# zlib-ng/minizip-ng

Measured on NVIDIA H100. Metric: deflate_l1_crc32_input_throughput, higher is better.
Workload: dtype u8

## Files before the change

minizip-ng_b200/csrc/deflate_kernel.cuh:

```cuda
#ifndef MZ_DEFLATE_KERNEL_CUH
#define MZ_DEFLATE_KERNEL_CUH

#include "mzcuda_common.cuh"

namespace mzc {

constexpr int DF_THREADS = 512;
constexpr int DF_WARPS = DF_THREADS / 32;
constexpr int DF_CHUNK_MAX = 65536;
constexpr int DF_UNIT = 32768;
constexpr int DF_SB = DF_UNIT;
constexpr int DF_SPAN = 8;
constexpr int DF_BATCH = DF_THREADS * DF_SPAN;
constexpr int DF_NBATCH = DF_UNIT / DF_BATCH;
constexpr int DF_MINMATCH = 4;
constexpr int DF_LOCKLEN = 8;
constexpr int DF_HASH_BITS = 13;
constexpr int DF_HASH_ENTRIES = 1 << DF_HASH_BITS;
constexpr int DF_STAGE_WORDS = DF_UNIT / 4 + 64;
constexpr int DF_HDR_WORDS = 96;

constexpr uint32_t DF_FLAG_FINAL = 1u;
constexpr uint32_t DF_FLAG_DICT = 2u;

constexpr int DF_OFF_IN = 0;
constexpr int DF_OFF_HASH = DF_OFF_IN + DF_UNIT + 64;
constexpr int DF_OFF_STAGE = DF_OFF_HASH;
constexpr int DF_OFF_REC = DF_OFF_HASH + DF_STAGE_WORDS * 4;
constexpr int DF_OFF_SPN = DF_OFF_REC + DF_NBATCH * DF_THREADS * 8;
constexpr int DF_SPAN_BYTES = DF_NBATCH * DF_THREADS * 10;
constexpr int DF_OFF_HIST = DF_OFF_REC + DF_SPAN_BYTES;
constexpr int DF_OFF_HIST2 = DF_OFF_HIST + (288 + 32) * 4;
constexpr int DF_OFF_CODE = DF_OFF_HIST2 + 256 * 4;
constexpr int DF_OFF_LENS = DF_OFF_CODE + (288 + 32) * 4;
constexpr int DF_OFF_BITS = DF_OFF_LENS + (288 + 32);
constexpr int DF_OFF_SCAN = DF_OFF_BITS + (288 + 32);
constexpr int DF_OFF_BB = DF_OFF_SCAN + 256 * 4;
constexpr int DF_OFF_MISC = DF_OFF_BB + 512 * 4;
constexpr int DF_OFF_SINK = DF_OFF_MISC + 32 * 4 + 16;
constexpr int DF_OFF_LSYM = DF_OFF_SINK + 32 * 4;
constexpr int DF_SMEM_BYTES = DF_OFF_LSYM + 256 * 2;
constexpr uint32_t DF_ZERO_SYM = 286;
static_assert(DF_HASH_ENTRIES * 4 <= DF_STAGE_WORDS * 4, "hash fits the staging region");
constexpr int DFH_PREV = 32768;
constexpr int DFH_HASH_BITS = 14;
constexpr int DFH_OFF_HASH = (DF_SMEM_BYTES + 15) & ~15;
constexpr int DFH_SMEM_BYTES = DFH_PREV + DFH_OFF_HASH + (4 << DFH_HASH_BITS);
static_assert(DFH_SMEM_BYTES <= 227 * 1024, "shared memory budget of the history variant");
static_assert(DF_SMEM_BYTES <= 113 * 1024, "shared memory budget for two CTAs per SM");

enum { MISC_CHUNK = 3, MISC_CARRY = 8  };

struct DeflateParams {
    const uint8_t *in;
    const uint64_t *in_off;
    const uint32_t *in_len;
    const uint8_t *flags;
    uint64_t total_len;
    uint32_t chunk_size;
    uint32_t nchunks;
    uint32_t last_flags;
    int32_t level;
    uint8_t *out;
    uint64_t slot_stride;
    uint32_t *out_len;
    uint32_t *work_counter;
};

__host__ __device__ inline uint64_t deflate_slot_bound(uint32_t chunk_size) {
    return (((uint64_t)chunk_size + 12ull * ((chunk_size + DF_SB - 1) / DF_SB + 1) + 64 + 15) & ~15ull);
}

__device__ __forceinline__ void length_symbol(uint32_t len, uint32_t &sym, uint32_t &ebits, uint32_t &eval) {
    const uint32_t l = len - 3;
    const uint32_t msb = 31u - (uint32_t)__clz((int)(l | 4u));
    uint32_t e = msb - 2;
    uint32_t sy = 4 * (e + 1) + ((l >> e) & 3u);
    uint32_t ev = l & ((1u << e) - 1u);
    sy = l < 8 ? l : sy;
    const bool top = len == 258;
    sym = top ? 28u : sy;
    ebits = top ? 0u : e;
    eval = top ? 0u : ev;
}
__device__ __forceinline__ void dist_symbol0(uint32_t d, uint32_t &sym, uint32_t &ebits) {
    uint32_t m = 31u - (uint32_t)__clz((int)(d | 1u));
    ebits = m > 0 ? m - 1 : 0u;
    sym = 2 * m + ((d >> ebits) & 1u);
}
__device__ __forceinline__ uint32_t len_extra_bits(uint32_t lsym) { return (lsym < 8 || lsym >= 28) ? 0u : (lsym >> 2) - 1; }
__device__ __forceinline__ uint32_t dist_extra_bits(uint32_t dsym) { return dsym < 4 ? 0u : (dsym >> 1) - 1; }

__device__ __forceinline__ uint32_t stage_word(uint32_t base, uint32_t pos, uint32_t k4) { return base + __umulhi(pos, 1u << 27) * k4; }

__device__ __forceinline__ void stage_put(uint32_t *stage, uint32_t pos, uint32_t v, uint32_t n) {
    if (n == 0) return;
    if (n < 32) v &= (1u << n) - 1;
    uint32_t w = pos >> 5, s = pos & 31;
    atomicOr(&stage[w], v << s);
    if (s + n > 32) atomicOr(&stage[w + 1], v >> (32 - s));
}

__device__ __forceinline__ void stage_or(const Smem &sm, uint32_t pos, uint32_t v, uint32_t n) {
    const uint32_t sh = pos & 31u, wa = DF_OFF_STAGE + ((pos >> 5) << 2);
    sm.red_or32(wa, v << sh);
    if (sh + n > 32) sm.red_or32(wa + 4, v >> (32 - sh));
}

struct BitWriter {
    Smem sm;
    uint64_t acc;
    uint32_t nb, wa;
    __device__ __forceinline__ void init(const Smem &s, uint32_t bitoff) {
        sm = s; wa = DF_OFF_STAGE + (bitoff >> 5) * 4; nb = bitoff & 31; acc = 0;
    }
    __device__ __forceinline__ void put(uint32_t v, uint32_t n) {
        acc |= (uint64_t)v << nb;
        nb += n;
        if (nb >= 32) {
            sm.red_or32(wa, (uint32_t)acc);
            acc >>= 32; nb -= 32; wa += 4;
        }
    }
    __device__ __forceinline__ uint32_t bitpos() const { return ((wa - (uint32_t)DF_OFF_STAGE) << 3) + nb; }
    __device__ __forceinline__ void finish() {
        if (nb > 0) sm.red_or32(wa, (uint32_t)acc);
        if (nb > 32) sm.red_or32(wa + 4, (uint32_t)(acc >> 32));
    }
};

__device__ inline uint32_t block_excl_sum(uint32_t v, uint32_t *scan, uint32_t &total) {
    uint32_t incl = warp_incl_sum(v);
    if (lane_id() == 31) scan[warp_id()] = incl;
    __syncthreads();
    if (warp_id() == 0) {
        uint32_t w = lane_id() < (unsigned)DF_WARPS ? scan[lane_id()] : 0u;
        uint32_t wi = warp_incl_sum(w);
        scan[32 + lane_id()] = wi - w;
        if (lane_id() == 31) scan[31] = wi;
    }
    __syncthreads();
    uint32_t res = scan[32 + warp_id()] + incl - v;
    total = scan[31];
    __syncthreads();
    return res;
}

enum { DF_PH_LOAD, DF_PH_PARSE, DF_PH_M0, DF_PH_COVER, DF_PH_T_M1, DF_PH_D, DF_PH_E_SCAN, DF_PH_F_M3, DF_PH_FLUSH, DF_PH_UNITS,
       DF_PH_D_STATS, DF_PH_D_SWEEP1, DF_PH_D_SWEEP2, DF_PH_D_KRAFT, DF_PH_D_CANON, DF_PH_D_PASSES, DF_PH_COLS = DF_PH_D_PASSES + 8 };
constexpr int DF_PH_ROWS = 1024;
#if defined(MZ_DF_PHASES) && !defined(MZ_EMU)
__device__ unsigned long long g_df_phases[DF_PH_ROWS][DF_PH_COLS];
#define DF_PHASE_BEGIN(t) unsigned long long t = clock64()
#define DF_PHASE(t, ph)                                                                        \
    do {                                                                                       \
        if (threadIdx.x == 0 && blockIdx.x < (unsigned)DF_PH_ROWS) {                           \
            const unsigned long long now_ = clock64();                                         \
            atomicAdd(&g_df_phases[blockIdx.x][ph], now_ - (t));                               \
            if ((ph) == DF_PH_LOAD) atomicAdd(&g_df_phases[blockIdx.x][DF_PH_UNITS], 1ull);   \
            (t) = now_;                                                                        \
        }                                                                                      \
    } while (0)
#define DF_PHASE_COUNT(col)                                                                                          \
    do {                                                                                                             \
        if (threadIdx.x == 0 && blockIdx.x < (unsigned)DF_PH_ROWS) atomicAdd(&g_df_phases[blockIdx.x][col], 1ull); \
    } while (0)
#else
#define DF_PHASE_BEGIN(t)
#define DF_PHASE(t, ph)
#define DF_PHASE_COUNT(col)
#endif

constexpr int DF_BB_THREADS = 320;
enum { BB_STAT = 0 , BB_KRAFT = 8 , BB_SLACK = 136 ,
       BB_CNTW = 144 ,
       BB_NZ = 464 , BB_ST = 474 ,
       BB_HSUM = 484 , BB_HDRBITS = 494  };

constexpr uint64_t CL_LENS = 0x12ddad91b725bb4ull;
constexpr uint64_t CL_CODE_LO = 0x840013930ef3c6ull, CL_CODE_HI = 0xd5c7fdf6cb149ull;
constexpr uint64_t CL_ORDER57 = 0x1b6d6db248db92dull;
__device__ __forceinline__ uint32_t cl_len(uint32_t s) { return (uint32_t)(CL_LENS >> (3 * s)) & 7u; }
__device__ __forceinline__ uint32_t cl_code(uint32_t s) {
    return s < 10 ? (uint32_t)(CL_CODE_LO >> (6 * s)) & 63u : (uint32_t)(CL_CODE_HI >> (6 * (s - 10))) & 63u;
}

__device__ __forceinline__ void bb_count_lengths(uint32_t *cntw_row, uint32_t L, unsigned lane, unsigned &m) {
    if (lane < 16) cntw_row[lane] = 0;
    __syncwarp();
    m = __match_any_sync(MZ_FULL_MASK, L);
    if (L > 0 && lane == (unsigned)(__ffs((int)m) - 1)) cntw_row[L] = (uint32_t)__popc(m);
    __syncwarp();
}

__device__ inline void block_build_codes(const uint32_t *hist_ll, const uint32_t *hist_lit2, const uint32_t *hist_d, uint8_t *lens_ll, uint8_t *lens_d,
                                         uint32_t *code_ll, uint32_t *code_d, uint8_t *bits_ll, uint8_t *bits_d, uint32_t *bb,
                                         uint32_t *stage, uint32_t hdrpos, uint32_t bfinal) {
    const uint32_t tid = threadIdx.x;
    const unsigned lane = lane_id(), w = warp_id();
    const int a = tid < 288 ? 0 : (tid < 320 ? 1 : 2);
    const uint32_t sym = a == 0 ? tid : tid - 288;
    const uint32_t nsym = a == 0 ? 286u : 30u;
    const int M = 15;
    const uint32_t one = 1u << M;
    const uint32_t w0 = a == 0 ? 0u : 9u;
    uint32_t c = (a < 2 && sym < nsym) ? (a == 0 ? hist_ll[sym] + (sym < 256 ? hist_lit2[sym] : 0u) : hist_d[sym]) : 0u;
    DF_PHASE_BEGIN(d_t);

    if (tid < 144) bb[tid] = (tid == BB_STAT + 2 || tid == BB_STAT + 6) ? 0xffffffffu : 0u;
    bar_sync(1, DF_BB_THREADS);
    if (a < 2) {
        uint32_t used_w = __reduce_add_sync(MZ_FULL_MASK, c ? 1u : 0u);
        uint32_t tot_w = __reduce_add_sync(MZ_FULL_MASK, c);
        uint32_t first_w = __reduce_min_sync(MZ_FULL_MASK, c ? sym : 0xffffffffu);
        if (lane == 0) {
            atomicAdd(&bb[BB_STAT + a * 4 + 0], used_w);
            atomicAdd(&bb[BB_STAT + a * 4 + 1], tot_w);
            atomicMin(&bb[BB_STAT + a * 4 + 2], first_w);
        }
    }
    bar_sync(1, DF_BB_THREADS);
    DF_PHASE(d_t, DF_PH_D_STATS);
    float ideal = 0.f;
    if (a < 2) {
        uint32_t used = bb[BB_STAT + a * 4 + 0], total = bb[BB_STAT + a * 4 + 1], fu = bb[BB_STAT + a * 4 + 2];
        if (used < 2) {
            uint32_t d0 = used == 0 ? 0u : (fu == 0 ? 1u : 0u);
            uint32_t d1 = used == 0 ? 1u : d0;
            if ((sym == d0 || sym == d1) && c == 0) c = 1;
            total += 2 - used;
        }
        if (c) ideal = __log2f((float)total) - __log2f((float)c);
// ... 130 lines not shown
        if (a == 0) {
            const uint32_t eb = sym >= 257 ? len_extra_bits(sym - 257) : 0u;
            lens_ll[sym] = (uint8_t)L;
            code_ll[sym] = cw | (eb << 20);
            bits_ll[sym] = (uint8_t)(L + eb);
        } else {
            lens_d[sym] = (uint8_t)L;
            code_d[sym] = cw;
            bits_d[sym] = (uint8_t)(L + dist_extra_bits(sym));
        }
    }
    const unsigned nz = __ballot_sync(MZ_FULL_MASK, L != 0);
    if (lane == 0) bb[BB_NZ + w] = nz;
    bar_sync(1, DF_BB_THREADS);
    DF_PHASE(d_t, DF_PH_D_CANON);
    const uint32_t hlit = 256u + 32u - (uint32_t)__clz((int)bb[BB_NZ + 8]);
    const uint32_t hdw = bb[BB_NZ + 9];
    const uint32_t hdist = hdw ? 32u - (uint32_t)__clz((int)hdw) : 1u;
    const uint32_t nlen = a == 0 ? hlit : hdist;
    const bool valid = sym < nlen;
    const uint32_t prevL = sym == 0 ? 0xffu : (a == 0 ? lens_ll[sym - 1] : lens_d[sym - 1]);
    const unsigned st = __ballot_sync(MZ_FULL_MASK, (valid && prevL != L) || sym == nlen);
    if (lane == 0) bb[BB_ST + w] = st;
    bar_sync(1, DF_BB_THREADS);
    uint32_t nb = 0, val = 0;
    if (valid) {
        uint32_t m = st & (0xffffffffu >> (31u - lane)), ww = w;
        while (m == 0) m = bb[BB_ST + --ww];
        const uint32_t s0 = (ww - w0) * 32u + 31u - (uint32_t)__clz((int)m);
        m = lane == 31 ? 0u : st & (0xfffffffeu << lane);
        ww = w;
        while (m == 0) m = bb[BB_ST + ++ww];
        const uint32_t e0 = (ww - w0) * 32u + (uint32_t)__ffs((int)m) - 1u;
        const uint32_t k = sym - s0, R = e0 - s0;
        uint32_t cs = L, ev = 0, eb = 0;
        bool tok = true;
        if (L == 0) {
            const uint32_t full = (R / 138u) * 138u, rem = R - full;
            if (k < full) { tok = k % 138u == 0; cs = 18; ev = 127; eb = 7; }
            else if (rem >= 11) { tok = k == full; cs = 18; ev = rem - 11; eb = 7; }
            else if (rem >= 3) { tok = k == full; cs = 17; ev = rem - 3; eb = 3; }
        } else if (k > 0) {
            const uint32_t k1 = k - 1, rest = R - 1, full = (rest / 6u) * 6u, rem = rest - full;
            if (k1 < full) { tok = k1 % 6u == 0; cs = 16; ev = 3; eb = 2; }
            else if (rem >= 3) { tok = k1 == full; cs = 16; ev = rem - 3; eb = 2; }
        }
        if (tok) {
            const uint32_t cl = cl_len(cs);
            nb = cl + eb;
            val = cl_code(cs) | (ev << cl);
        }
    }
    const uint32_t incl = warp_incl_sum(nb);
    if (lane == 31) bb[BB_HSUM + w] = incl;
    bar_sync(1, DF_BB_THREADS);
    uint32_t off = incl - nb, total = 0;
    for (uint32_t ww = 0; ww < 10; ww++) {
        const uint32_t t = bb[BB_HSUM + ww];
        off += ww < w ? t : 0u;
        total += t;
    }
    if (nb) stage_put(stage, hdrpos + 17 + 57 + off, val, nb);
    if (tid == 0) {
        stage_put(stage, hdrpos, bfinal | (2u << 1) | ((hlit - 257u) << 3) | ((hdist - 1u) << 8) | (15u << 13), 17);
        bb[BB_HDRBITS] = 17 + 57 + total;
    }
    if (tid == 32) stage_put(stage, hdrpos + 17, (uint32_t)CL_ORDER57, 32);
    if (tid == 64) stage_put(stage, hdrpos + 17 + 32, (uint32_t)(CL_ORDER57 >> 32), 25);
}

__device__ __forceinline__ uint32_t extend_match8(const Smem &sm, uint32_t c, uint32_t q, uint32_t maxlen) {
    uint32_t len = 8;
    while (len < maxlen) {
        uint32_t x = sm.ld32u(DF_OFF_IN, q + len) ^ sm.ld32u(DF_OFF_IN, c + len);
        if (x) {
            len += (uint32_t)(__ffs((int)x) - 1) >> 3;
            break;
        }
        len += 4;
    }
    return len < maxlen ? len : maxlen;
}

__device__ __forceinline__ uint32_t opaque4() { return blockDim.x / (uint32_t)(DF_THREADS / 4); }

template <bool HIST>
__device__ __forceinline__ uint32_t hash_addr(uint32_t v, uint32_t k4) {
    return (HIST ? DFH_OFF_HASH : DF_OFF_HASH) + __umulhi(v * 2654435761u, 1u << (HIST ? DFH_HASH_BITS : DF_HASH_BITS)) * k4;
}

__device__ __forceinline__ uint32_t rec_len(uint32_t r) { uint32_t l = (r >> 3) & 255u; return l ? l + 3 : 0u; }

__device__ __forceinline__ uint32_t fin_len(uint32_t m) { return ((m >> 4) & 255u) + 3u; }
__device__ __forceinline__ uint32_t fin_dist(uint32_t m) { return ((m >> 12) & 0x7fffu) + 1u; }
template <bool ONEM>
__device__ __forceinline__ void span_classify(const Smem &sm, uint32_t A, uint32_t B, uint32_t q0, uint32_t cover, uint32_t &F, uint32_t &MA,
                                              uint32_t &MB) {
    const uint32_t lit = (A >> 26) | ((B >> 26) << 6);
    const uint32_t crel = cover > q0 ? cover - q0 : 0u;
    const uint32_t cr8 = crel < 8 ? crel : 8u;
    uint32_t ex = 0;
    MA = MB = 0;
#pragma unroll
    for (int r = 0; r < (ONEM ? 1 : 2); r++) {
        const uint32_t R = r == 0 ? A : B;
        const uint32_t j = R & 7u, end = j + rec_len(R);
        const uint32_t s = j > crel ? j : crel;
        const uint32_t Lf = (end > s ? end : s) - s;
        const uint32_t P = (s < 8u ? s : 8u) & 7u;
        const uint32_t M = Lf >= 3 ? (((Lf << 4) + (0x80000000u - (3u << 4))) | P | ((R << 1) & (0x7fffu << 12))) : 0u;
        if (r == 0) MA = M;
        else MB = M;
        ex = Lf - 1u < 2u ? Lf : ex;
    }
    F = ((lit >> cr8) << cr8) | (ex << 8);
    if (ex) {
        const uint32_t p = DF_OFF_IN + q0 + crel;
        F |= sm.ld8(p) << 16;
        if (ex == 2) F |= sm.ld8(p + 1) << 24;
    }
}

__device__ __forceinline__ uint32_t match_symbols(const Smem &sm, uint32_t M) {
    uint32_t ds, db;
    const uint32_t lsv = sm.ld16(DF_OFF_LSYM + ((M >> 3) & 0x1feu));
    const uint32_t d = fin_dist(M) - 1;
    dist_symbol0(d, ds, db);
    sm.red_add32(DF_OFF_HIST + (257u + (lsv & 31u)) * 4, 1u);
    sm.red_add32(DF_OFF_HIST + (288u + ds) * 4, 1u);
    return 0x80000000u | ((M & 7u) << 28) | ((d & ((1u << db) - 1u)) << 15) | (ds << 10) | lsv;
}
__device__ __forceinline__ uint32_t match_bits(const Smem &sm, uint32_t M) {
    const uint32_t n = sm.ld8(DF_OFF_BITS + 257u + (M & 31u)) + sm.ld8(DF_OFF_BITS + 288u + ((M >> 10) & 31u));
    return M ? n : 0u;
}
__device__ __forceinline__ void put_match_bits(const Smem &sm, uint32_t pos, uint32_t M) {
    const uint32_t cwl = sm.ld32(DF_OFF_CODE + (257u + (M & 31u)) * 4);
    const uint32_t cwd = sm.ld32(DF_OFF_CODE + (288u + ((M >> 10) & 31u)) * 4);
    const uint32_t cl = (cwl >> 16) & 15u, cd = (cwd >> 16) & 15u;
    const uint32_t v1 = (cwl & 0x7fffu) | (((M >> 5) & 31u) << cl);
    const uint32_t n1 = cl + ((cwl >> 20) & 15u);
    const uint32_t v2 = (cwd & 0x7fffu) | (((M >> 15) & 0x1fffu) << cd);
    const uint64_t V = (uint64_t)v1 | ((uint64_t)v2 << n1);
    const uint32_t lo = (uint32_t)V, hi = (uint32_t)(V >> 32);
    const uint32_t wa = stage_word(DF_OFF_STAGE, pos, opaque4());
    const uint32_t w0 = __funnelshift_l(0u, lo, pos), w1 = __funnelshift_l(lo, hi, pos), w2 = __funnelshift_l(hi, 0u, pos);
    sm.red_or32(wa, w0);
    sm.red_or32(wa + 4, w1);
    if (w2) sm.red_or32(wa + 8, w2);
}

__device__ __forceinline__ uint32_t nth_parked(const uint32_t (&bm)[DF_NBATCH], uint32_t k, uint32_t warp) {
    uint32_t r = k, word = 0, bsel = 0;
    bool found = false;
#pragma unroll
    for (int b = 0; b < DF_NBATCH; b++) {
        const uint32_t c = (uint32_t)__popc(bm[b]);
        const bool here = !found && r < c;
        word = here ? bm[b] : word;
        bsel = here ? (uint32_t)b : bsel;
        found = found || here;
        r -= found ? 0u : c;
    }
    uint32_t base = 0;
#pragma unroll
    for (int st = 16; st; st >>= 1) {
// ... 88 lines not shown
            __syncthreads();
        }

        for (uint32_t u = 0; u < nunits; u++) {
            const uint32_t ustart = u * DF_UNIT;
            const uint32_t ulen = (ustart + DF_UNIT < len) ? (uint32_t)DF_UNIT : len - ustart;
            const uint8_t *gin = P.in + off + ustart;
            const bool last_unit = u == nunits - 1;
            const uint32_t nb = (ulen + DF_BATCH - 1) / DF_BATCH;

            const uint32_t len16 = ulen & ~15u;
            bool bulk = false;
#ifndef MZ_EMU
            bulk = (((uintptr_t)gin) & 15) == 0 && len16 > 0;
            if (bulk && tid == 0) {
                fence_proxy_async();
                mbar_expect_tx(s_bar, len16);
                tma_load_1d(s_in, gin, len16, s_bar);
            }
#endif
            if (!bulk) {
                if ((((uintptr_t)gin) & 15) == 0) {
                    for (uint32_t i = tid * 16; i < len16; i += DF_THREADS * 16) *(uint4 *)(s_in + i) = ldg_stream((const uint4 *)(gin + i));
                } else {
                    for (uint32_t i = tid; i < len16; i += DF_THREADS) s_in[i] = gin[i];
                }
            }
            for (uint32_t i = len16 + tid; i < ulen; i += DF_THREADS) s_in[i] = gin[i];
            for (uint32_t i = ulen + tid; i < ((ulen + 63) & ~15u) + 16 && i < DF_UNIT + 64; i += DF_THREADS) s_in[i] = 0;
            if (P.level != 0) {
                if (!HIST) {
                    for (uint32_t i = tid; i < DF_HASH_ENTRIES / 4; i += DF_THREADS) sm.st128(DF_OFF_HASH + i * 16, ~0u, ~0u, ~0u, ~0u);
                } else if (u == 0) {
                    for (uint32_t i = tid; i < (1u << DFH_HASH_BITS) / 4; i += DF_THREADS) sm.st128(DFH_OFF_HASH + i * 16, ~0u, ~0u, ~0u, ~0u);
                    if (dict) {
                        const uint8_t *gp = P.in + off - DFH_PREV;
                        if ((((uintptr_t)gp) & 15) == 0) {
                            for (uint32_t i = tid * 16; i < (uint32_t)DFH_PREV; i += DF_THREADS * 16) *(uint4 *)(smem - DFH_PREV + i) = ldg_stream((const uint4 *)(gp + i));
                        } else {
                            for (uint32_t i = tid; i < (uint32_t)DFH_PREV; i += DF_THREADS) smem[(int)i - DFH_PREV] = gp[i];
                        }
                    }
                } else {
                    for (uint32_t i = tid; i < (1u << DFH_HASH_BITS) / 4; i += DF_THREADS) {
                        uint4 e = *(const uint4 *)(smem + DFH_OFF_HASH + i * 16);
                        e.x = (e.x != ~0u && (e.x & 0xffffu) >= (uint32_t)DFH_PREV) ? e.x + 0x78000u : ~0u;
                        e.y = (e.y != ~0u && (e.y & 0xffffu) >= (uint32_t)DFH_PREV) ? e.y + 0x78000u : ~0u;
                        e.z = (e.z != ~0u && (e.z & 0xffffu) >= (uint32_t)DFH_PREV) ? e.z + 0x78000u : ~0u;
                        e.w = (e.w != ~0u && (e.w & 0xffffu) >= (uint32_t)DFH_PREV) ? e.w + 0x78000u : ~0u;
                        *(uint4 *)(smem + DFH_OFF_HASH + i * 16) = e;
                    }
                }
            }
#ifndef MZ_EMU
            if (bulk) {
                mbar_wait(s_bar, bar_phase);
                bar_phase ^= 1;
            }
#endif
            __syncthreads();
            if (HIST && P.level != 0 && u == 0 && dict) {
#pragma unroll 1
                for (uint32_t b = 0; b < (uint32_t)DF_NBATCH; b++) {
                    const uint32_t p0 = b * DF_BATCH + tid * DF_SPAN;
                    const uint2 x = sm.ld64((uint32_t)(DF_OFF_IN - DFH_PREV) + p0);
                    const uint32_t y = sm.ld32((uint32_t)(DF_OFF_IN - DFH_PREV) + p0 + 8);
                    const uint32_t key0 = ((15u - b) << 16) | p0;
#pragma unroll
                    for (int j = 0; j < 8; j++) {
                        const uint32_t v = j == 0 ? x.x : (j < 4 ? __funnelshift_r(x.x, x.y, 8 * j) : (j == 4 ? x.y : __funnelshift_r(x.y, y, 8 * (j - 4))));
                        sm.red_min32(hash_addr<true>(v, 4u), key0 + j);
                    }
                }
                __syncthreads();
            }
            DF_PHASE(ph_t, DF_PH_LOAD);

            uint32_t fF[DF_NBATCH], fA[DF_NBATCH];
            bool stored = (P.level == 0);
            const uint32_t bfinal = (last_unit && (flags & DF_FLAG_FINAL)) ? 1u : 0u;
            uint32_t tokbits = 0;

            if (P.level != 0) {
#pragma unroll 1
                for (uint32_t b = 0; b < nb; b++) {
                    const uint32_t q0 = b * DF_BATCH + tid * DF_SPAN;
                    uint32_t v[12], ha[8], lc[8];
                    const uint32_t k4 = opaque4();
                    {
                        const uint2 x = sm.ld64(DF_OFF_IN + q0), y = sm.ld64(DF_OFF_IN + q0 + 8);
                        v[0] = x.x; v[4] = x.y; v[8] = y.x;
#pragma unroll
                        for (int k = 1; k < 4; k++) {
                            v[k] = __funnelshift_r(x.x, x.y, 8 * k);
                            v[4 + k] = __funnelshift_r(x.y, y.x, 8 * k);
                            v[8 + k] = __funnelshift_r(y.x, y.y, 8 * k);
                        }
                    }
#pragma unroll
                    for (int j = 0; j < 8; j++) {
                        ha[j] = hash_addr<HIST>(v[j], k4);
                        if (j % STRIDE == 0) lc[j] = sm.ld32(ha[j]);
                    }
                    const uint32_t nvalid = ulen > q0 ? (ulen - q0 < 8 ? ulen - q0 : 8u) : 0u;
                    __syncthreads();
                    {
                        const uint32_t key0 = ((uint32_t)(DF_NBATCH - 1 - b) << 16) | (CUR + q0);
#pragma unroll
                        for (int j = 0; j < 8; j++) sm.red_min32(ha[j], key0 + j);
                    }
                    __syncthreads();
#pragma unroll
                    for (int j = 0; j < 8; j++) {
                        if (j % STRIDE != 0) {
                            lc[j] = 0;
                            continue;
                        }
                        const uint32_t cn = sm.ld32(ha[j]) & 0xffffu;
                        const uint32_t pq = CUR + q0 + j;
                        const uint32_t c = cn < pq ? cn : (lc[j] & 0xffffu);
                        const uint32_t ca = DF_OFF_IN - CUR + (c & ~3u);
                        const uint32_t w0 = sm.ld32(ca), w1 = sm.ld32(ca + 4), w2 = sm.ld32(ca + 8);
                        const uint32_t s = c << 3;
                        const uint32_t x0 = __funnelshift_r(w0, w1, s) ^ v[j];
                        const uint32_t x1 = __funnelshift_r(w1, w2, s) ^ v[j + 4];
                        const bool reach = c < pq && (!HIST || c >= q0 + j);
                        const uint32_t l = (reach && x0 == 0) ? 4u + ((uint32_t)__clz((int)__brev(x1)) >> 3) : 0u;
                        lc[j] = l | ((pq - c - 1u) << 4);
                    }
                    if (q0 + 16 > ulen) {
#pragma unroll
                        for (int j = 0; j < 8; j += STRIDE) {
                            const uint32_t room = ulen > q0 + j ? ulen - (q0 + j) : 0u;
                            uint32_t l = lc[j] & 15u;
                            l = l < room ? l : room;
                            lc[j] = (lc[j] & ~15u) | (l >= (uint32_t)DF_MINMATCH ? l : 0u);
                        }
                    }
                    uint32_t nxt = 0, lit = 0, mA = 0, mB = 0, span_end = 0;
                    if (STRIDE == 2 && !LAZY && !ONEM) {
                        uint32_t endA = 0, endB = 0;
#pragma unroll
                        for (int j = 6; j >= 0; j -= 2) {
                            const uint32_t l = lc[j] & 15u;
                            const uint32_t rec = (uint32_t)j | ((l - 3) << 3) | ((lc[j] >> 4) << 11);
                            mA = l ? rec : mA;
                            endA = l ? (uint32_t)j + l : endA;
                        }
#pragma unroll
                        for (int j = 6; j >= 2; j -= 2) {
                            const uint32_t l = lc[j] & 15u;
                            const uint32_t rec = (uint32_t)j | ((l - 3) << 3) | ((lc[j] >> 4) << 11);
                            const bool nextm = l != 0 && (uint32_t)j >= endA;
                            mB = nextm ? rec : mB;
                            endB = nextm ? (uint32_t)j + l : endB;
                        }
                        lit = ~(((1u << endA) - (1u << (mA & 7u))) | ((1u << endB) - (1u << (mB & 7u)))) & 0xffu;
                        span_end = mB ? endB : endA;
                    } else {
#pragma unroll
                        for (int j = 0; j < 8; j++) {
                            const bool take = nxt == (uint32_t)j;
                            if (j % STRIDE == 0) {
                                const uint32_t l = lc[j] & 15u;
                                bool ism = take && l >= (uint32_t)DF_MINMATCH;
                                if (LAZY && STRIDE == 1 && j < 7) ism = ism && !((lc[j + 1] & 15u) > l);
                                const uint32_t rec = (uint32_t)j | ((l - 3) << 3) | ((lc[j] >> 4) << 11);
                                const bool first = mA == 0;
                                if (ONEM) ism = ism && first;
                                mA = (ism && first) ? rec : mA;
                                if (!ONEM) mB = (ism && !first) ? rec : mB;
                                lit |= (take && !ism) ? (1u << j) : 0u;
                                nxt = ism ? (uint32_t)j + l : (take ? (uint32_t)j + 1u : nxt);
                            } else {
                                lit |= take ? (1u << j) : 0u;
                                nxt = take ? (uint32_t)j + 1u : nxt;
                            }
                        }
                        const uint32_t last = mB ? mB : mA;
                        span_end = last ? (last & 7u) + rec_len(last) : 0u;
                    }
                    lit &= (1u << nvalid) - 1u;
                    {
                        const uint32_t last = mB ? mB : mA;
                        const uint32_t capped = __ballot_sync(MZ_FULL_MASK, ((last >> 3) & 255u) == (uint32_t)(DF_LOCKLEN - 3));
                        if (lane == 0) s_scan[b * DF_WARPS + warp] = capped;
                        sm.st64(DF_OFF_REC + (b * DF_THREADS + tid) * 8, mA | ((lit & 63u) << 26), mB | ((lit >> 6) << 26));
                        sm.st16(DF_OFF_SPN + (b * DF_THREADS + tid) * 2, ((last & 7u) << 9) | span_end);
                    }
                }
                DF_PHASE(ph_t, DF_PH_PARSE);
                {
                    __syncwarp();
                    uint32_t bmX[DF_NBATCH], totX = 0;
#pragma unroll
                    for (int b = 0; b < DF_NBATCH; b++) {
                        bmX[b] = (uint32_t)b < nb ? s_scan[b * DF_WARPS + warp] : 0u;
                        totX += (uint32_t)__popc(bmX[b]);
                    }
                    for (uint32_t k0 = 0; k0 < totX; k0 += 32) {
                        const uint32_t sidx = nth_parked(bmX, k0 + lane, warp);
                        if (sidx != 0xffffffffu) {
                            const uint2 r = sm.ld64(DF_OFF_REC + sidx * 8);
                            const bool second = (r.y & 0x03ffffffu) != 0;
                            const uint32_t w = second ? r.y : r.x, last = w & 0x03ffffffu;
                            const uint32_t j = last & 7u, q = sidx * DF_SPAN + j, c = q - ((last >> 11) & 0x7fffu) - 1u;
                            uint32_t maxlen = ulen - q;
                            maxlen = maxlen < 258 ? maxlen : 258u;
                            uint32_t l = 0, cb = c;
                            if (q >= 4) {
                                const uint32_t a0 = sm.ld32u(DF_OFF_IN, q), a1 = sm.ld32u(DF_OFF_IN, q + 4);
                                const bool p4 = a0 == a1, p3 = __funnelshift_r(a0, a1, 24) == a0;
                                if (p4 || p3) {
                                    uint32_t cn = c;
                                    if (p4) {
                                        if (a0 == sm.ld32u(DF_OFF_IN, q - 4)) cn = q - 4;
                                        if (a0 == sm.ld32u(DF_OFF_IN, q - 2)) cn = q - 2;
                                        if (a0 == sm.ld32u(DF_OFF_IN, q - 1)) cn = q - 1;
                                    } else if (a0 == sm.ld32u(DF_OFF_IN, q - 3) && a1 == sm.ld32u(DF_OFF_IN, q + 1)) {
                                        cn = q - 3;
                                    }
                                    if (cn != c) {
                                        const uint32_t pd = q - cn;
                                        if (q >= 12u && (sidx & 31u) != 0u && sm.ld32u(DF_OFF_IN, q - 8) == sm.ld32u(DF_OFF_IN, q - 8 - pd) &&
                                            sm.ld32u(DF_OFF_IN, q - 4) == sm.ld32u(DF_OFF_IN, q - 4 - pd)) {
                                            const uint32_t left = ulen - sidx * DF_SPAN, nval = left < 8u ? left : 8u;
                                            const uint32_t lit = ((r.x >> 26) | ((r.y >> 26) << 6) | (0xffu << j)) & ((1u << nval) - 1u);
                                            const uint32_t mA = second ? (r.x & 0x03ffffffu) : 0u;
                                            sm.st64(DF_OFF_REC + sidx * 8, mA | ((lit & 63u) << 26), (lit >> 6) << 26);
                                            sm.st16(DF_OFF_SPN + sidx * 2, mA ? ((mA & 7u) << 9) | ((mA & 7u) + rec_len(mA)) : 0u);
                                            continue;
                                        }
                                        l = extend_match8(sm, cn, q, maxlen);
                                        cb = cn;
                                    }
                                }
                            }
                            if (l < 64u && l < maxlen) {
                                const uint32_t lf = extend_match8(sm, c, q, maxlen);
                                if (lf > l) {
                                    l = lf;
                                    cb = c;
                                }
                            }
                            sm.st32(DF_OFF_REC + sidx * 8 + (second ? 4u : 0u), (w & ~((255u << 3) | (0x7fffu << 11))) | ((l - 3) << 3) | ((q - cb - 1u) << 11));
                            sm.st16(DF_OFF_SPN + sidx * 2, (j << 9) | (j + l));
                        }
                    }
                }
                __syncthreads();
                DF_PHASE(ph_t, DF_PH_M0);

                for (uint32_t i = tid; i < DF_STAGE_WORDS / 4; i += DF_THREADS) {
                    if (i == 0) sm.st128(DF_OFF_STAGE, s_misc[MISC_CARRY], s_misc[MISC_CARRY + 1], s_misc[MISC_CARRY + 2], s_misc[MISC_CARRY + 3]);
                    else sm.st128(DF_OFF_STAGE + i * 16, 0, 0, 0, 0);
                }
                for (uint32_t i = tid; i < 288 + 32 + 256; i += DF_THREADS) s_hist_ll[i] = 0;

                {
                    uint32_t se[8];
                    if (tid * 8 < nb * DF_THREADS) {
                        const uint4 q = *(const uint4 *)(smem + DF_OFF_SPN + tid * 16);
                        se[0] = q.x & 0xffffu; se[1] = q.x >> 16; se[2] = q.y & 0xffffu; se[3] = q.y >> 16;
                        se[4] = q.z & 0xffffu; se[5] = q.z >> 16; se[6] = q.w & 0xffffu; se[7] = q.w >> 16;
                    } else {
#pragma unroll
                        for (int k = 0; k < 8; k++) se[k] = 0;
                    }
                    const uint32_t p0 = tid * 64;
                    uint32_t tmax = 0;
#pragma unroll
                    for (int k = 0; k < 8; k++) {
                        const uint32_t e = se[k] ? p0 + 8 * k + (se[k] & 511u) : 0u;
                        tmax = tmax > e ? tmax : e;
                    }
                    const uint32_t incl = warp_incl_max(tmax);
                    uint32_t cin = __shfl_up_sync(MZ_FULL_MASK, incl, 1);
                    if (lane == 0) cin = 0;
                    if (lane == 31) s_scan[warp] = incl;
                    __syncthreads();
                    {
                        const uint32_t w = (lane < (unsigned)DF_WARPS && lane < warp) ? s_scan[lane] : 0u;
                        const uint32_t base = __reduce_max_sync(MZ_FULL_MASK, w);
                        cin = cin > base ? cin : base;
                    }
                    uint32_t run = cin, drop = 0, pcv = 0, pendk = 0;
                    bool alive = false;
                    uint32_t cv[8];
#pragma unroll
                    for (int k = 0; k < 8; k++) {
                        const uint32_t q0 = p0 + 8 * k;
                        const uint32_t ms = q0 + (se[k] >> 9), me = q0 + (se[k] & 511u);
                        const bool fc = run >= q0 + 8;
                        const bool strad = se[k] != 0 && ms < run && me > run;
                        const bool takes = fc && strad && alive && ms <= pcv;
                        drop |= takes ? 1u << pendk : 0u;
                        cv[k] = takes ? pcv : run;
                        pcv = (fc && strad && !takes) ? run : pcv;
                        pendk = (fc && strad) ? (uint32_t)k : pendk;
                        alive = fc && (strad || alive);
                        run = (se[k] != 0 && me > run) ? me : run;
                    }
#pragma unroll
                    for (int k = 0; k < 8; k++) cv[k] = ((drop >> k) & 1u) ? 0xffffu : cv[k];
                    *(uint4 *)(smem + DF_OFF_SPN + tid * 16) = make_uint4(cv[0] | (cv[1] << 16), cv[2] | (cv[3] << 16), cv[4] | (cv[5] << 16), cv[6] | (cv[7] << 16));
                }
                __syncthreads();
                DF_PHASE(ph_t, DF_PH_COVER);

                const uint32_t hist_lit = sm.addr((lane & 1u) ? (uint32_t)DF_OFF_HIST2 : (uint32_t)DF_OFF_HIST);
                const uint32_t k4 = opaque4();
                const uint32_t sink = sm.addr(DF_OFF_SINK + lane * 4);
                uint32_t bmB[DF_NBATCH];
#pragma unroll
                for (int b = 0; b < DF_NBATCH; b++) {
                    uint32_t F = 0, MA = 0, MB = 0;
                    bmB[b] = 0;
                    if ((uint32_t)b < nb) {
                        const uint32_t sidx = (uint32_t)b * DF_THREADS + tid;
                        const uint32_t q0 = sidx * DF_SPAN;
                        const uint2 r = sm.ld64(DF_OFF_REC + sidx * 8);
                        const uint32_t cover = sm.ld16(DF_OFF_SPN + sidx * 2);
                        span_classify<ONEM>(sm, r.x, r.y, q0, cover, F, MA, MB);
                        const uint32_t ex = (F >> 8) & 3u;
                        if (ex) {
                            sm.red_add32_a(hist_lit + ((F >> 16) & 0xffu) * 4, 1u);
                            if (ex == 2) sm.red_add32_a(hist_lit + (F >> 24) * 4, 1u);
                        }
                        const uint2 x = sm.ld64(DF_OFF_IN + q0);
// ... 218 lines not shown
```

minizip-ng_b200/csrc/mzcuda_common.cuh:

```cuda
#ifndef MZCUDA_COMMON_CUH
#define MZCUDA_COMMON_CUH

#include <stdint.h>

#ifdef MZ_EMU
#include "cuda_emu.h"
#define MZ_DYN_SMEM(name) uint8_t *name = emu_dyn_smem
#ifndef MZ_EMU_ACCESS
#define MZ_EMU_ACCESS(p, bytes, kind, newval)
#define MZ_EMU_PREEMPT()
#endif
#else
#include <cuda_runtime.h>
#define MZ_LAUNCH(kernel, grid, block, smem, stream, ...) kernel<<<(grid), (block), (smem), (stream)>>>(__VA_ARGS__)
#define MZ_DYN_SMEM(name) extern __shared__ __align__(128) uint8_t name[]
#endif

#define MZ_FULL_MASK 0xffffffffu

namespace mzc {

__device__ __forceinline__ unsigned lane_id() { return threadIdx.x & 31; }
__device__ __forceinline__ unsigned warp_id() { return threadIdx.x >> 5; }

__device__ __forceinline__ uint32_t load32u(const uint8_t *base, uint32_t p) {
    const uint32_t *w = (const uint32_t *)(base + (p & ~3u));
    return __funnelshift_r(w[0], w[1], (p & 3u) * 8u);
}

__device__ __forceinline__ uint4 ldg_stream(const uint4 *p) {
#ifdef MZ_EMU
    MZ_EMU_PREEMPT();
    return *p;
#else
    uint4 r;
    asm volatile("ld.global.nc.L1::no_allocate.v4.u32 {%0,%1,%2,%3}, [%4];" : "=r"(r.x), "=r"(r.y), "=r"(r.z), "=r"(r.w) : "l"(p));
    return r;
#endif
}


struct Smem {
#ifdef MZ_EMU
    uint8_t *b;
    __device__ __forceinline__ void init(uint8_t *base) { b = base; }
    __device__ __forceinline__ uint8_t *p(uint32_t off) const { return b + (int32_t)off; }
    __device__ __forceinline__ uint32_t ld32(uint32_t off) const { MZ_EMU_ACCESS(p(off), 4, EMU_ACC_READ, nullptr); return *(const uint32_t *)p(off); }
    __device__ __forceinline__ uint32_t ld16(uint32_t off) const { MZ_EMU_ACCESS(p(off), 2, EMU_ACC_READ, nullptr); return *(const uint16_t *)p(off); }
    __device__ __forceinline__ uint32_t ld8(uint32_t off) const { MZ_EMU_ACCESS(p(off), 1, EMU_ACC_READ, nullptr); return *p(off); }
    __device__ __forceinline__ void st32(uint32_t off, uint32_t v) const { MZ_EMU_ACCESS(p(off), 4, EMU_ACC_WRITE, &v); *(uint32_t *)p(off) = v; }
    __device__ __forceinline__ void st16(uint32_t off, uint32_t v) const {
        const uint16_t h = (uint16_t)v;
        MZ_EMU_ACCESS(p(off), 2, EMU_ACC_WRITE, &h);
        *(uint16_t *)p(off) = h;
    }
    __device__ __forceinline__ void red_or32(uint32_t off, uint32_t v) const { MZ_EMU_ACCESS(p(off), 4, EMU_ACC_ATOMIC, nullptr); *(uint32_t *)p(off) |= v; }
    __device__ __forceinline__ void red_add32(uint32_t off, uint32_t v) const { MZ_EMU_ACCESS(p(off), 4, EMU_ACC_ATOMIC, nullptr); *(uint32_t *)p(off) += v; }
    __device__ __forceinline__ void red_min32(uint32_t off, uint32_t v) const {
        MZ_EMU_ACCESS(p(off), 4, EMU_ACC_ATOMIC, nullptr);
        uint32_t *q = (uint32_t *)p(off);
        if (v < *q) *q = v;
    }
    __device__ __forceinline__ void st16_if(bool c, uint32_t off, uint32_t v) const { if (c) st16(off, v); }
    __device__ __forceinline__ void red_add32_if(bool c, uint32_t off, uint32_t v) const { if (c) red_add32(off, v); }
    __device__ __forceinline__ void red_or32_if(bool c, uint32_t off, uint32_t v) const { if (c) red_or32(off, v); }
    __device__ __forceinline__ uint2 ld64(uint32_t off) const { MZ_EMU_ACCESS(p(off), 8, EMU_ACC_READ, nullptr); return *(const uint2 *)p(off); }
    __device__ __forceinline__ void st64(uint32_t off, uint32_t x, uint32_t y) const {
        const uint2 v = make_uint2(x, y);
        MZ_EMU_ACCESS(p(off), 8, EMU_ACC_WRITE, &v);
        *(uint2 *)p(off) = v;
    }
    __device__ __forceinline__ void st128(uint32_t off, uint32_t x, uint32_t y, uint32_t z, uint32_t w) const {
        const uint4 v = make_uint4(x, y, z, w);
        MZ_EMU_ACCESS(p(off), 16, EMU_ACC_WRITE, &v);
        *(uint4 *)p(off) = v;
    }
    __device__ __forceinline__ uint32_t addr(uint32_t off) const { return off; }
    __device__ __forceinline__ uint32_t ld32_a(uint32_t a) const { return ld32(a); }
    __device__ __forceinline__ uint32_t ld8_a(uint32_t a) const { return ld8(a); }
    __device__ __forceinline__ void red_or32_a(uint32_t a, uint32_t v) const { red_or32(a, v); }
    __device__ __forceinline__ void red_add32_a(uint32_t a, uint32_t v) const { red_add32(a, v); }
#else
    uint32_t b;
    __device__ __forceinline__ void init(uint8_t *base) {
        b = (uint32_t)__cvta_generic_to_shared(base);
        asm volatile("" : "+r"(b));
    }
    __device__ __forceinline__ uint32_t ld32(uint32_t off) const {
        uint32_t v;
        asm volatile("ld.shared.u32 %0, [%1];" : "=r"(v) : "r"(b + off));
        return v;
    }
    __device__ __forceinline__ uint32_t ld16(uint32_t off) const {
        uint32_t v;
        asm volatile("ld.shared.u16 %0, [%1];" : "=r"(v) : "r"(b + off));
        return v;
    }
    __device__ __forceinline__ uint32_t ld8(uint32_t off) const {
        uint32_t v;
        asm volatile("ld.shared.u8 %0, [%1];" : "=r"(v) : "r"(b + off));
        return v;
    }
    __device__ __forceinline__ void st32(uint32_t off, uint32_t v) const { asm volatile("st.shared.u32 [%0], %1;" ::"r"(b + off), "r"(v) : "memory"); }
    __device__ __forceinline__ void st16(uint32_t off, uint32_t v) const { asm volatile("st.shared.u16 [%0], %1;" ::"r"(b + off), "r"(v) : "memory"); }
    __device__ __forceinline__ void red_or32(uint32_t off, uint32_t v) const { asm volatile("red.shared.or.b32 [%0], %1;" ::"r"(b + off), "r"(v) : "memory"); }
    __device__ __forceinline__ void red_add32(uint32_t off, uint32_t v) const { asm volatile("red.shared.add.u32 [%0], %1;" ::"r"(b + off), "r"(v) : "memory"); }
    __device__ __forceinline__ void red_min32(uint32_t off, uint32_t v) const { asm volatile("red.shared.min.u32 [%0], %1;" ::"r"(b + off), "r"(v) : "memory"); }
    __device__ __forceinline__ void st16_if(bool p, uint32_t off, uint32_t v) const {
        asm volatile("{\n.reg .pred q;\nsetp.ne.u32 q, %2, 0;\n@q st.shared.u16 [%0], %1;\n}" ::"r"(b + off), "r"(v), "r"((uint32_t)p) : "memory");
    }
    __device__ __forceinline__ void red_add32_if(bool p, uint32_t off, uint32_t v) const {
        asm volatile("{\n.reg .pred q;\nsetp.ne.u32 q, %2, 0;\n@q red.shared.add.u32 [%0], %1;\n}" ::"r"(b + off), "r"(v), "r"((uint32_t)p) : "memory");
    }
    __device__ __forceinline__ void red_or32_if(bool p, uint32_t off, uint32_t v) const {
        asm volatile("{\n.reg .pred q;\nsetp.ne.u32 q, %2, 0;\n@q red.shared.or.b32 [%0], %1;\n}" ::"r"(b + off), "r"(v), "r"((uint32_t)p) : "memory");
    }
    __device__ __forceinline__ uint2 ld64(uint32_t off) const {
        uint2 v;
        asm volatile("ld.shared.v2.u32 {%0,%1}, [%2];" : "=r"(v.x), "=r"(v.y) : "r"(b + off));
        return v;
    }
    __device__ __forceinline__ void st64(uint32_t off, uint32_t x, uint32_t y) const { asm volatile("st.shared.v2.u32 [%0], {%1,%2};" ::"r"(b + off), "r"(x), "r"(y) : "memory"); }
    __device__ __forceinline__ void st128(uint32_t off, uint32_t x, uint32_t y, uint32_t z, uint32_t w) const {
        asm volatile("st.shared.v4.u32 [%0], {%1,%2,%3,%4};" ::"r"(b + off), "r"(x), "r"(y), "r"(z), "r"(w) : "memory");
    }
    __device__ __forceinline__ uint32_t addr(uint32_t off) const { return b + off; }
    __device__ __forceinline__ uint32_t ld32_a(uint32_t a) const {
        uint32_t v;
        asm volatile("ld.shared.u32 %0, [%1];" : "=r"(v) : "r"(a));
        return v;
    }
    __device__ __forceinline__ uint32_t ld8_a(uint32_t a) const {
        uint32_t v;
        asm volatile("ld.shared.u8 %0, [%1];" : "=r"(v) : "r"(a));
        return v;
    }
    __device__ __forceinline__ void red_or32_a(uint32_t a, uint32_t v) const { asm volatile("red.shared.or.b32 [%0], %1;" ::"r"(a), "r"(v) : "memory"); }
    __device__ __forceinline__ void red_add32_a(uint32_t a, uint32_t v) const { asm volatile("red.shared.add.u32 [%0], %1;" ::"r"(a), "r"(v) : "memory"); }
#endif
    __device__ __forceinline__ uint32_t ld32u(uint32_t off, uint32_t p) const {
        uint32_t a = off + (p & ~3u);
        return __funnelshift_r(ld32(a), ld32(a + 4), (p & 3u) * 8u);
    }
};

__device__ __forceinline__ void bar_sync(int id, int nthreads) {
#ifdef MZ_EMU
    emu_named_barrier(id, nthreads);
#else
    asm volatile("bar.sync %0, %1;" ::"r"(id), "r"(nthreads) : "memory");
#endif
}

__device__ __forceinline__ uint32_t warp_incl_sum(uint32_t v) {
#pragma unroll
    for (int d = 1; d < 32; d <<= 1) {
        uint32_t n = __shfl_up_sync(MZ_FULL_MASK, v, d);
        if (lane_id() >= (unsigned)d) v += n;
    }
    return v;
}

__device__ __forceinline__ uint32_t warp_incl_max(uint32_t v) {
#pragma unroll
    for (int d = 1; d < 32; d <<= 1) {
        uint32_t n = __shfl_up_sync(MZ_FULL_MASK, v, d);
        if (lane_id() >= (unsigned)d) v = v > n ? v : n;
    }
    return v;
}

__device__ __forceinline__ uint32_t shl_clamp(uint32_t v, uint32_t s) {
#ifdef MZ_EMU
    return s >= 32u ? 0u : v << s;
#else
    uint32_t r;
    asm("shl.b32 %0, %1, %2;" : "=r"(r) : "r"(v), "r"(s));
    return r;
#endif
}
__device__ __forceinline__ uint32_t shr_clamp(uint32_t v, uint32_t s) {
#ifdef MZ_EMU
    return s >= 32u ? 0u : v >> s;
#else
    uint32_t r;
    asm("shr.u32 %0, %1, %2;" : "=r"(r) : "r"(v), "r"(s));
    return r;
#endif
}
#define MZ_BYTE(x, k) __byte_perm((x), 0u, 0x4440u + (k))

#ifndef MZ_EMU
// ... 39 lines not shown
```

Measured before the change: 150.1.

## Compact capped-span lists and pack match records directly in parse loop

```diff
diff --git a/minizip-ng_b200/csrc/deflate_kernel.cuh b/minizip-ng_b200/csrc/deflate_kernel.cuh
--- a/minizip-ng_b200/csrc/deflate_kernel.cuh
+++ b/minizip-ng_b200/csrc/deflate_kernel.cuh
@@ -40,6 +40,8 @@
 constexpr int DF_OFF_SINK = DF_OFF_MISC + 32 * 4 + 16;
 constexpr int DF_OFF_LSYM = DF_OFF_SINK + 32 * 4;
 constexpr int DF_SMEM_BYTES = DF_OFF_LSYM + 256 * 2;
+constexpr int DF_OFF_CAPL = DF_OFF_HIST;
+static_assert(DF_OFF_CAPL + DF_WARPS * DF_NBATCH * 32 <= DF_OFF_SCAN, "capped-span lists fit in front of the scan scratch");
 constexpr uint32_t DF_ZERO_SYM = 286;
 static_assert(DF_HASH_ENTRIES * 4 <= DF_STAGE_WORDS * 4, "hash fits the staging region");
 constexpr int DFH_PREV = 32768;
@@ -147,7 +149,8 @@
 }
 
 enum { DF_PH_LOAD, DF_PH_PARSE, DF_PH_M0, DF_PH_COVER, DF_PH_T_M1, DF_PH_D, DF_PH_E_SCAN, DF_PH_F_M3, DF_PH_FLUSH, DF_PH_UNITS,
-       DF_PH_D_STATS, DF_PH_D_SWEEP1, DF_PH_D_SWEEP2, DF_PH_D_KRAFT, DF_PH_D_CANON, DF_PH_D_PASSES, DF_PH_COLS = DF_PH_D_PASSES + 8 };
+       DF_PH_D_STATS, DF_PH_D_SWEEP1, DF_PH_D_SWEEP2, DF_PH_D_KRAFT, DF_PH_D_CANON, DF_PH_D_PASSES,
+       DF_PH_P_A = DF_PH_D_PASSES + 8, DF_PH_P_B, DF_PH_P_C, DF_PH_M_INDEX, DF_PH_M_NEAR, DF_PH_M_EXTEND, DF_PH_COLS };
 constexpr int DF_PH_ROWS = 1024;
 #if defined(MZ_DF_PHASES) && !defined(MZ_EMU)
 __device__ unsigned long long g_df_phases[DF_PH_ROWS][DF_PH_COLS];
@@ -444,6 +447,16 @@
     return len < maxlen ? len : maxlen;
 }
 
+__device__ __forceinline__ uint32_t sel_u32(bool p, uint32_t a, uint32_t b) {
+#ifdef MZ_EMU
+    return p ? a : b;
+#else
+    uint32_t r;
+    asm("{\n.reg .pred q;\nsetp.ne.u32 q, %3, 0;\nselp.b32 %0, %1, %2, q;\n}" : "=r"(r) : "r"(a), "r"(b), "r"((uint32_t)p));
+    return r;
+#endif
+}
+
 __device__ __forceinline__ uint32_t opaque4() { return blockDim.x / (uint32_t)(DF_THREADS / 4); }
 
 template <bool HIST>
@@ -698,6 +711,8 @@
             uint32_t tokbits = 0;
 
             if (P.level != 0) {
+                DF_PHASE_BEGIN(p_t);
+                uint32_t ncap = 0;
 #pragma unroll 1
                 for (uint32_t b = 0; b < nb; b++) {
                     const uint32_t q0 = b * DF_BATCH + tid * DF_SPAN;
@@ -720,57 +735,46 @@
                     }
                     const uint32_t nvalid = ulen > q0 ? (ulen - q0 < 8 ? ulen - q0 : 8u) : 0u;
                     __syncthreads();
-                    {
-                        const uint32_t key0 = ((uint32_t)(DF_NBATCH - 1 - b) << 16) | (CUR + q0);
-#pragma unroll
-                        for (int j = 0; j < 8; j++) sm.red_min32(ha[j], key0 + j);
-                    }
+                    DF_PHASE(p_t, DF_PH_P_A);
+                    const uint32_t key0 = ((uint32_t)(DF_NBATCH - 1 - b) << 16) | (CUR + q0);
+#pragma unroll
+                    for (int j = 0; j < 8; j++) sm.red_min32(ha[j], key0 + j);
                     __syncthreads();
+                    DF_PHASE(p_t, DF_PH_P_B);
 #pragma unroll
                     for (int j = 0; j < 8; j++) {
                         if (j % STRIDE != 0) {
                             lc[j] = 0;
                             continue;
                         }
-                        const uint32_t cn = sm.ld32(ha[j]) & 0xffffu;
-                        const uint32_t pq = CUR + q0 + j;
-                        const uint32_t c = cn < pq ? cn : (lc[j] & 0xffffu);
-                        const uint32_t ca = DF_OFF_IN - CUR + (c & ~3u);
+                        const uint32_t kp = key0 + j, kn = sm.ld32(ha[j]);
+                        const uint32_t ck = kn < kp ? kn : lc[j];
+                        const uint32_t c = HIST ? ck & 0xffffu : ck;
+                        const uint32_t ca = DF_OFF_IN - CUR + (c & 0xfffcu);
                         const uint32_t w0 = sm.ld32(ca), w1 = sm.ld32(ca + 4), w2 = sm.ld32(ca + 8);
                         const uint32_t s = c << 3;
                         const uint32_t x0 = __funnelshift_r(w0, w1, s) ^ v[j];
                         const uint32_t x1 = __funnelshift_r(w1, w2, s) ^ v[j + 4];
-                        const bool reach = c < pq && (!HIST || c >= q0 + j);
-                        const uint32_t l = (reach && x0 == 0) ? 4u + ((uint32_t)__clz((int)__brev(x1)) >> 3) : 0u;
-                        lc[j] = l | ((pq - c - 1u) << 4);
+                        const bool reach = HIST ? c < CUR + q0 + j && c >= q0 + j : ck != 0xffffffffu;
+                        const uint32_t l3 = ((uint32_t)__clz((int)__brev(x1)) & ~7u) + 8u;
+                        lc[j] = sel_u32(reach && x0 == 0, (((kp - ck - 1u) << 11) & (0x7fffu << 11)) + l3 + (uint32_t)j, 0u);
                     }
                     if (q0 + 16 > ulen) {
 #pragma unroll
                         for (int j = 0; j < 8; j += STRIDE) {
                             const uint32_t room = ulen > q0 + j ? ulen - (q0 + j) : 0u;
-                            uint32_t l = lc[j] & 15u;
-                            l = l < room ? l : room;
-                            lc[j] = (lc[j] & ~15u) | (l >= (uint32_t)DF_MINMATCH ? l : 0u);
+                            const uint32_t l = rec_len(lc[j]);
+                            lc[j] = l >= (uint32_t)DF_MINMATCH && l > room ? (room >= (uint32_t)DF_MINMATCH ? lc[j] - ((l - room) << 3) : 0u) : lc[j];
                         }
                     }
                     uint32_t nxt = 0, lit = 0, mA = 0, mB = 0, span_end = 0;
                     if (STRIDE == 2 && !LAZY && !ONEM) {
-                        uint32_t endA = 0, endB = 0;
-#pragma unroll
-                        for (int j = 6; j >= 0; j -= 2) {
-                            const uint32_t l = lc[j] & 15u;
-                            const uint32_t rec = (uint32_t)j | ((l - 3) << 3) | ((lc[j] >> 4) << 11);
-                            mA = l ? rec : mA;
-                            endA = l ? (uint32_t)j + l : endA;
-                        }
-#pragma unroll
-                        for (int j = 6; j >= 2; j -= 2) {
-                            const uint32_t l = lc[j] & 15u;
-                            const uint32_t rec = (uint32_t)j | ((l - 3) << 3) | ((lc[j] >> 4) << 11);
-                            const bool nextm = l != 0 && (uint32_t)j >= endA;
-                            mB = nextm ? rec : mB;
-                            endB = nextm ? (uint32_t)j + l : endB;
-                        }
+#pragma unroll
+                        for (int j = 6; j >= 0; j -= 2) mA = lc[j] ? lc[j] : mA;
+                        const uint32_t endA = (mA & 7u) + rec_len(mA);
+#pragma unroll
+                        for (int j = 6; j >= 2; j -= 2) mB = lc[j] && (uint32_t)j >= endA ? lc[j] : mB;
+                        const uint32_t endB = (mB & 7u) + rec_len(mB);
                         lit = ~(((1u << endA) - (1u << (mA & 7u))) | ((1u << endB) - (1u << (mB & 7u)))) & 0xffu;
                         span_end = mB ? endB : endA;
                     } else {
@@ -778,10 +782,9 @@
                         for (int j = 0; j < 8; j++) {
                             const bool take = nxt == (uint32_t)j;
                             if (j % STRIDE == 0) {
-                                const uint32_t l = lc[j] & 15u;
-                                bool ism = take && l >= (uint32_t)DF_MINMATCH;
-                                if (LAZY && STRIDE == 1 && j < 7) ism = ism && !((lc[j + 1] & 15u) > l);
-                                const uint32_t rec = (uint32_t)j | ((l - 3) << 3) | ((lc[j] >> 4) << 11);
+                                const uint32_t rec = lc[j], l = rec_len(rec);
+                                bool ism = take && rec != 0;
+                                if (LAZY && STRIDE == 1 && j < 7) ism = ism && !(((lc[j + 1] >> 3) & 255u) > ((rec >> 3) & 255u));
                                 const bool first = mA == 0;
                                 if (ONEM) ism = ism && first;
                                 mA = (ism && first) ? rec : mA;
@@ -799,24 +802,25 @@
                     lit &= (1u << nvalid) - 1u;
                     {
                         const uint32_t last = mB ? mB : mA;
-                        const uint32_t capped = __ballot_sync(MZ_FULL_MASK, ((last >> 3) & 255u) == (uint32_t)(DF_LOCKLEN - 3));
-                        if (lane == 0) s_scan[b * DF_WARPS + warp] = capped;
+                        const bool cap = ((last >> 3) & 255u) == (uint32_t)(DF_LOCKLEN - 3);
+                        const uint32_t capped = __ballot_sync(MZ_FULL_MASK, cap);
+                        sm.st8_if(cap, DF_OFF_CAPL + warp * 256u + ncap + (uint32_t)__popc(capped & ((1u << lane) - 1u)), (b << 5) | lane);
+                        ncap += (uint32_t)__popc(capped);
                         sm.st64(DF_OFF_REC + (b * DF_THREADS + tid) * 8, mA | ((lit & 63u) << 26), mB | ((lit >> 6) << 26));
                         sm.st16(DF_OFF_SPN + (b * DF_THREADS + tid) * 2, ((last & 7u) << 9) | span_end);
                     }
+                    DF_PHASE(p_t, DF_PH_P_C);
                 }
                 DF_PHASE(ph_t, DF_PH_PARSE);
                 {
+                    DF_PHASE_BEGIN(m_t);
                     __syncwarp();
-                    uint32_t bmX[DF_NBATCH], totX = 0;
-#pragma unroll
-                    for (int b = 0; b < DF_NBATCH; b++) {
-                        bmX[b] = (uint32_t)b < nb ? s_scan[b * DF_WARPS + warp] : 0u;
-                        totX += (uint32_t)__popc(bmX[b]);
-                    }
-                    for (uint32_t k0 = 0; k0 < totX; k0 += 32) {
-                        const uint32_t sidx = nth_parked(bmX, k0 + lane, warp);
-                        if (sidx != 0xffffffffu) {
+                    for (uint32_t k0 = 0; k0 < ncap; k0 += 32) {
+                        const uint32_t k = k0 + lane;
+                        const uint32_t e = k < ncap ? sm.ld8(DF_OFF_CAPL + warp * 256u + k) : 0u;
+                        const uint32_t sidx = (e >> 5) * (uint32_t)DF_THREADS + warp * 32u + (e & 31u);
+                        DF_PHASE(m_t, DF_PH_M_INDEX);
+                        if (k < ncap) {
                             const uint2 r = sm.ld64(DF_OFF_REC + sidx * 8);
                             const bool second = (r.y & 0x03ffffffu) != 0;
                             const uint32_t w = second ? r.y : r.x, last = w & 0x03ffffffu;
@@ -852,6 +856,7 @@
                                     }
                                 }
                             }
+                            DF_PHASE(m_t, DF_PH_M_NEAR);
                             if (l < 64u && l < maxlen) {
                                 const uint32_t lf = extend_match8(sm, c, q, maxlen);
                                 if (lf > l) {
@@ -861,6 +866,7 @@
                             }
                             sm.st32(DF_OFF_REC + sidx * 8 + (second ? 4u : 0u), (w & ~((255u << 3) | (0x7fffu << 11))) | ((l - 3) << 3) | ((q - cb - 1u) << 11));
                             sm.st16(DF_OFF_SPN + sidx * 2, (j << 9) | (j + l));
+                            DF_PHASE(m_t, DF_PH_M_EXTEND);
                         }
                     }
                 }
diff --git a/minizip-ng_b200/csrc/mzcuda_common.cuh b/minizip-ng_b200/csrc/mzcuda_common.cuh
--- a/minizip-ng_b200/csrc/mzcuda_common.cuh
+++ b/minizip-ng_b200/csrc/mzcuda_common.cuh
@@ -62,6 +62,12 @@
         if (v < *q) *q = v;
     }
     __device__ __forceinline__ void st16_if(bool c, uint32_t off, uint32_t v) const { if (c) st16(off, v); }
+    __device__ __forceinline__ void st8_if(bool c, uint32_t off, uint32_t v) const {
+        if (!c) return;
+        const uint8_t h = (uint8_t)v;
+        MZ_EMU_ACCESS(p(off), 1, EMU_ACC_WRITE, &h);
+        *p(off) = h;
+    }
     __device__ __forceinline__ void red_add32_if(bool c, uint32_t off, uint32_t v) const { if (c) red_add32(off, v); }
     __device__ __forceinline__ void red_or32_if(bool c, uint32_t off, uint32_t v) const { if (c) red_or32(off, v); }
     __device__ __forceinline__ uint2 ld64(uint32_t off) const { MZ_EMU_ACCESS(p(off), 8, EMU_ACC_READ, nullptr); return *(const uint2 *)p(off); }
@@ -108,6 +114,9 @@
     __device__ __forceinline__ void red_min32(uint32_t off, uint32_t v) const { asm volatile("red.shared.min.u32 [%0], %1;" ::"r"(b + off), "r"(v) : "memory"); }
     __device__ __forceinline__ void st16_if(bool p, uint32_t off, uint32_t v) const {
         asm volatile("{\n.reg .pred q;\nsetp.ne.u32 q, %2, 0;\n@q st.shared.u16 [%0], %1;\n}" ::"r"(b + off), "r"(v), "r"((uint32_t)p) : "memory");
+    }
+    __device__ __forceinline__ void st8_if(bool p, uint32_t off, uint32_t v) const {
+        asm volatile("{\n.reg .pred q;\nsetp.ne.u32 q, %2, 0;\n@q st.shared.u8 [%0], %1;\n}" ::"r"(b + off), "r"(v), "r"((uint32_t)p) : "memory");
     }
     __device__ __forceinline__ void red_add32_if(bool p, uint32_t off, uint32_t v) const {
         asm volatile("{\n.reg .pred q;\nsetp.ne.u32 q, %2, 0;\n@q red.shared.add.u32 [%0], %1;\n}" ::"r"(b + off), "r"(v), "r"((uint32_t)p) : "memory");
```

After: 155.6 (median of 6 runs). +3.7%, better.
